# ponkrshnan/VI-HMC

Hardware: AMD Instinct MI355X
Metric: leapfrog-steps/sec/GPU (grad evals/sec) + ESS/sec, DeepONet VI-HMC (higher is better)
Workload: dtype fp32

## Files before the change

### vi-hmc_amd/csrc/vihmc_bwd_bf.hip

```cpp
#include "vihmc_internal.h"
#include "vihmc_bf16x6.h"
#include <type_traits>

namespace vihmc {

namespace {
using bf6::f32x4;
using bf6::bf16x8;
using bf6::bf16x4;
using bf6::split4;
using bf6::six;
using bf6::tr_frag;

constexpr int BB_SUB = BWD_SUB;
constexpr int BB_PITCH = bf6::PITCH;
constexpr int BB_PLANE = BB_SUB * BB_PITCH;
constexpr int BB_DP = 0;
constexpr int BB_HP = 3 * BB_PLANE;
constexpr int BB_DT = 6 * BB_PLANE;
constexpr int BB_BUF = BB_DT + BB_SUB * 16;
constexpr int BB_WPITCH = 224;
constexpr int BB_WPLANE = 100 * BB_WPITCH;
constexpr int BB_W = 2 * BB_BUF;
constexpr int BB_WT = BB_W + 3 * BB_WPLANE;
constexpr int BB_LDS = BB_WT + 100 * 16;
static_assert(BB_LDS <= 160 * 1024, "LDS");
static_assert(BB_BUF + 2 * BB_PLANE < 65536, "LDS store offsets fit the ds_write immediate");
constexpr int BB_THREADS = 1024;
constexpr int B2_HSLOTS = 2;

__device__ __forceinline__ int hslot(int r, int c4) { return c4 ^ ((r >> 2) & 3); }

__device__ __forceinline__ float act_grad_bf(int act, float h) {
#pragma clang fp contract(off)
    if (act == ACT_TANH) return 1.f - h * h;
    if (act == ACT_RELU) return h > 0.f ? 1.f : 0.f;
    return 1.f;
}
__device__ __forceinline__ float tanh_grad(float h) {
#pragma clang fp contract(off)
    return 1.f - h * h;
}
}

#if BB_STAMP
constexpr int BBS_WG = 16, BBS_SUB = 32, BBS_K = 6;
__device__ unsigned long long bb_stamps[BBS_WG][16][BBS_SUB][BBS_K];
__device__ unsigned long long bb_real[BBS_WG][2][2];
#define VIHMC_BB_STAMP(I, K)                                                                                  \
    __builtin_amdgcn_sched_barrier(0);                                                                        \
    if (samp && lane == 0 && (I) < BBS_SUB) bb_stamps[sidx][wave][(I)][(K)] = __builtin_amdgcn_s_memtime();   \
    __builtin_amdgcn_sched_barrier(0);
#else
#define VIHMC_BB_STAMP(I, K)
#endif
constexpr int BBS_NONE = 1 << 20;

__global__ __launch_bounds__(BB_THREADS, 1) void k_bwd_bf2(BwdArgs args) {
    extern __shared__ __attribute__((aligned(16))) unsigned char smw[];
    int b = blockIdx.x;
    const int per0 = args.C * args.p[0].n_wg;
    const bool second = b >= per0;
    const BwdProb P = second ? args.p[1] : args.p[0];
    if (second) b -= per0;
    const int c = b / P.n_wg;
    const int wg = b - c * P.n_wg;
    const int tid = threadIdx.x, wave = tid >> 6, lane = tid & 63, lr = lane & 15, lg = lane >> 4;
    const int NI4 = (P.n_in + 3) & ~3;
    const int hq4 = NI4 >> 2;
    const float* D = P.D + c * P.d_cs;
    const float* H = P.H + c * P.h_cs;
    const int r0 = wg * P.rows_per_wg;
    const int r1 = min(P.M, r0 + P.rows_per_wg);
    const int nsub = r1 > r0 ? (r1 - r0 + BB_SUB - 1) / BB_SUB : 0;
#if BB_STAMP
    const bool samp = second && P.has_dx && (b % 16) == 0 && b / 16 < BBS_WG;
    const int sidx = b / 16;
    if (samp && tid == 0) {
        bb_real[sidx][0][0] = __builtin_amdgcn_s_memtime();
        bb_real[sidx][0][1] = __builtin_amdgcn_s_memrealtime();
    }
#endif

    if (P.has_dx && wave < 12) {
        const float* WT = P.WT + c * P.wt_cs;
        constexpr int WTH = 768;
        constexpr int WSL = (100 * 25 + WTH - 1) / WTH;
        f32x4 wx[WSL];
#pragma unroll
        for (int v = 0; v < WSL; ++v) {
            const int idx = min(tid + WTH * v, P.n_in * 25 - 1);
            const int r = idx / 25, c4 = idx - r * 25;
            wx[v] = *reinterpret_cast<const f32x4*>(WT + (int64_t)r * P.ldw + 4 * c4);
        }
#pragma unroll
        for (int v = 0; v < WSL; ++v) {
            const int idx = tid + WTH * v;
            if (idx >= P.n_in * 25) break;
            const int r = idx / 25, c4 = idx - r * 25;
            bf16x4 p0, p1, p2;
            split4(wx[v], p0, p1, p2);
            unsigned char* o = smw + BB_W + r * BB_WPITCH + 8 * c4;
            *reinterpret_cast<bf16x4*>(o) = p0;
            *reinterpret_cast<bf16x4*>(o + BB_WPLANE) = p1;
            *reinterpret_cast<bf16x4*>(o + 2 * BB_WPLANE) = p2;
            if (c4 == 24) *reinterpret_cast<f32x4*>(smw + BB_WT + r * 16) = wx[v];
        }
    }

    if (wave >= 12) {
        const int g = __builtin_amdgcn_readfirstlane(wave - 12);
        {
            const int t = tid - 768;
            if (t < 2 * BB_SUB) {
                unsigned char* o = smw + (t >> 5) * BB_BUF + BB_HP + (t & 31) * BB_PITCH + 8 * hslot(t & 31, NI4 >> 2);
                *reinterpret_cast<unsigned short*>(o) = 0x3F80;
                *reinterpret_cast<unsigned short*>(o + BB_PLANE) = 0;
                *reinterpret_cast<unsigned short*>(o + 2 * BB_PLANE) = 0;
            }
        }
// ... 244 lines not shown
        const int tro = bf6::tr_lane_off(lr, lg);
        const int troh = (4 * lg + (lr >> 2)) * BB_PITCH + 8 * ((lr & 3) ^ lg);
        auto dw_run = [&](auto nt_c) __attribute__((always_inline)) {
            constexpr int NT = decltype(nt_c)::value;
            const int nt = NT ? NT : ntj;
            for (int i = 0; i < nsub; ++i) {
                __syncthreads();
                VIHMC_BB_STAMP(i, 0)
                const unsigned char* buf = smw + (i & 1) * BB_BUF;
                bf16x8 da[2][3], hb[2][3];
#pragma unroll
                for (int p = 0; p < 3; ++p) {
                    da[0][p] = tr_frag(buf + BB_DP + p * BB_PLANE, tro, 16 * rta);
                    da[1][p] = tr_frag(buf + BB_DP + p * BB_PLANE, tro, 16 * rtb);
                    hb[0][p] = tr_frag(buf + BB_HP + p * BB_PLANE, troh, 0);
                }
#pragma unroll
                for (int t = 0; t < 7; ++t) {
                    if (t >= nt) break;
                    if (t + 1 < nt) {
#pragma unroll
                        for (int p = 0; p < 3; ++p) hb[(t + 1) & 1][p] = tr_frag(buf + BB_HP + p * BB_PLANE, troh, 16 * (t + 1));
                    }
                    acc[0][t] = six(da[0], hb[t & 1], acc[0][t]);
                    if (t >= cb0 && t < cb1) acc[1][t] = six(da[1], hb[t & 1], acc[1][t]);
                }
#if BB_STAMP
                asm volatile("" :: "v"(acc[0][0]), "v"(acc[1][6]));
                VIHMC_BB_STAMP(i, 2)
#endif
            }
        };
        if (ntj == 7) dw_run(std::integral_constant<int, 7>{});
        else dw_run(std::integral_constant<int, 0>{});
        float* part = P.part + c * P.part_cs + (int64_t)wg * P.part_stride;
#pragma unroll
        for (int s2 = 0; s2 < 2; ++s2) {
            const int tn = s2 == 0 ? rta : rtb;
#pragma unroll
            for (int t = 0; t < 7; ++t) {
                if (t >= ntj || (s2 == 1 && (t < cb0 || t >= cb1))) continue;
                if (tn < 6 || lg == 0) *reinterpret_cast<f32x4*>(part + bwd_tile_off(tn, t, ntj, lane)) = acc[s2][t];
            }
        }
    }
#if BB_STAMP
    if (samp && tid == 0) {
        bb_real[sidx][1][0] = __builtin_amdgcn_s_memtime();
        bb_real[sidx][1][1] = __builtin_amdgcn_s_memrealtime();
    }
#endif
}

bool bwd_bf_ok(const BwdArgs& a) {
    for (int i = 0; i < a.nprob; ++i) {
        const BwdProb& p = a.p[i];
        if (p.n_out != 100 || ((p.n_in + 3) & ~3) >= 112 || (p.has_dx && p.n_in != 100)) return false;
        if ((p.ldd & 3) || (p.ldh & 3) || (p.has_dx && (p.ldw & 3)) || p.rows_per_wg % BWD_SUB) return false;
    }
    return true;
}

#if BB_STAMP
extern "C" int vihmc_debug_bb_stamps(void* stamps, size_t stamp_bytes, void* real, size_t real_bytes) {
    if (stamp_bytes != sizeof(bb_stamps) || real_bytes != sizeof(bb_real)) return -1;
    hipError_t e = hipMemcpyFromSymbol(stamps, HIP_SYMBOL(bb_stamps), stamp_bytes, 0, hipMemcpyDeviceToHost);
    if (e == hipSuccess) e = hipMemcpyFromSymbol(real, HIP_SYMBOL(bb_real), real_bytes, 0, hipMemcpyDeviceToHost);
    return (int)e;
}
#endif

hipError_t launch_bwd_bf(const BwdArgs& a, hipStream_t s) {
    if (!bwd_bf_ok(a)) return hipErrorInvalidValue;
    const int blocks = a.C * a.p[0].n_wg + (a.nprob > 1 ? a.C * a.p[1].n_wg : 0);
    hipLaunchKernelGGL(k_bwd_bf2, dim3(blocks), dim3(BB_THREADS), BB_LDS, s, a);
    return hipGetLastError();
}


}
```

### vi-hmc_amd/csrc/vihmc_internal.h

```cpp
#pragma once
#include <hip/hip_runtime.h>
#include <cstdint>
#include <vector>

#include "vihmc_diag.h"

namespace vihmc {

enum { ACT_ID = 0, ACT_TANH = 1, ACT_RELU = 2, ACT_SINE = 3 };

__device__ __forceinline__ float tanh_acc(float x) {
    const float ax = fabsf(x);
    const float u = x * x;
    float p = fmaf(u, -0.005816340912133455f, 0.020738132297992706f);
    p = fmaf(u, p, -0.053769949823617935f);
    p = fmaf(u, p, 0.13331805169582367f);
    p = fmaf(u, p, -0.33333295583724976f);
    const float small = fmaf(x * u, p, x);
    const float t = __builtin_amdgcn_exp2f(fmaf(ax, -2.885390043258667f, ax * -3.851926067000022e-08f));
    const float big = copysignf(fmaf(-2.f, t * __builtin_amdgcn_rcpf(1.f + t), 1.f), x);
    return ax < 0.625f ? small : big;
}
__device__ __forceinline__ float tanh_cr(float x) {
    const double a = fmin(fabs((double)x), 20.0);
// ... 17 lines not shown
    const double den = em + 2.0;
    const double rc = __builtin_amdgcn_rcp(den);
    const double y0 = em * rc;
    const double y = fma(fma(-y0, den, em), rc, y0);
    return copysignf((float)y, x);
}
enum { ACT_TANH_CR = 4 };
enum { MODE_FWD = 0, MODE_BWD = 1 };

constexpr int CONTRACT_OWN_PER_WG = 128;
constexpr int CONTRACT_QC = 16;
constexpr int CONTRACT_SPLIT_ROWS = 32;
constexpr int CONTRACT_SPLIT_BLOCK = 22528;
constexpr int ROWDOT_WAVES = 4;

struct RowdotProb {
    const float* A; int64_t a_cs; int32_t lda;
    const float* B; int64_t b_cs; int32_t ldb;
    float* O;       int64_t o_cs; int32_t ldo;
    const float* bias; int64_t bias_cs;
    const float* H; int64_t h_cs; int32_t ldh;
    int32_t M, Nn, K, act;
    int32_t tiles;
    int32_t ntiles;
    int32_t tpw;
};
struct RowdotArgs {
    RowdotProb p[2];
    int32_t nprob, C;
    int32_t ms0;
};



constexpr int BWD_SUB = 32;

constexpr int GATHER_SPLIT_MAX = 256;
struct BwdProb {
    const float* D;  int64_t d_cs;  int32_t ldd;
    const float* WT; int64_t wt_cs; int32_t ldw;
    const float* H;  int64_t h_cs;  int32_t ldh;
    float* Dout;     int64_t o_cs;
    float* part;     int64_t part_cs; int32_t part_stride;
    int32_t M, n_out, n_in, act, has_dx;
    int32_t rows_per_wg, n_wg;
};
struct BwdArgs {
    BwdProb p[2];
    int32_t nprob, C;
};
hipError_t launch_bwd(const BwdArgs& a, int nti, hipStream_t s);
bool bwd_bf_ok(const BwdArgs& a);
hipError_t launch_bwd_bf(const BwdArgs& a, hipStream_t s);

constexpr int BWD_CHAIN_MAXL = 12;
struct BwdChainLayer {
    const float* H; int64_t h_cs; int32_t ldh;
    int32_t n_in, n_out;
    int32_t act;
    int64_t part_off; int32_t part_stride;
};
struct BwdChainNet {
    BwdChainLayer L[BWD_CHAIN_MAXL];
    int32_t nl, M, n_wg;
    int32_t tanh_all;
    const float* D; int64_t d_cs; int32_t ldd;
    float* dwpart; int64_t dwpart_cs;
    const unsigned char* wtimg; int64_t wtimg_cs;
};
struct BwdChainArgs {
    BwdChainNet net[2];
    int32_t C;
};
bool bwd_chain_ok(const BwdChainArgs& a);
hipError_t launch_bwd_chain(const BwdChainArgs& a, hipStream_t s);
int bwd_chain_rows();

constexpr int GUARD_MAXC = 256;
struct ChainBits {
    uint32_t w[GUARD_MAXC / 32];
};
__host__ __device__ inline bool chain_bit(const ChainBits& b, int c) {
    return c < GUARD_MAXC && ((b.w[c >> 5] >> (c & 31)) & 1u) != 0u;
}

struct ContractProb {
    const float* Own; int64_t own_cs; int32_t ldown;
    const float* Q;   int64_t q_cs;   int32_t ldq;
    const float* Y;   int32_t ldy; int64_t y_cs;
    float* gout;      int64_t gout_cs; int32_t ldg;
    const float* b0;  int64_t b0_cs;
    float* out;       int64_t out_cs; int32_t ldout; int64_t out_chunk_stride;
    double* stats;    int64_t stats_cs;
    int32_t Mo, Mq, W;
    int32_t o_tiles, q_chunks, q_per_chunk;
    int32_t with_stats, write_s;
    int32_t load_g;
    int32_t masked;
    int32_t xcd_group;
    int32_t bf16x6;
    const unsigned char* qimg; int64_t qimg_cs;
    float gscale;
    int32_t sel; ChainBits bits;
};

constexpr int MOMENTS_TILE_N = 64;
// ... 256 lines not shown
```

### vi-hmc_amd/csrc/vihmc_plan.hip

```cpp
#include <algorithm>
#include <cmath>
#include <cstring>
#include <string>
#include <vector>

#include "vihmc.h"
#include "vihmc_internal.h"
#include <cstdlib>
#include <cstdio>

using namespace vihmc;

namespace {

thread_local std::string g_err;
constexpr size_t CANARY_BYTES = 4096;

int fail(const std::string& msg, int code = 1) {
    g_err = msg;
    return code;
}

#define HIPCHK(expr)                                                                              \
    do {                                                                                          \
// ... 103 lines not shown
    float* gT = nullptr;
    int64_t gT_cs = 0;
    int ldgT = 0;
    unsigned char* qsplitA = nullptr;
    int64_t qsplitA_cs = 0;
    unsigned char* qsplitB = nullptr;
    int64_t qsplitB_cs = 0;
    bool img_by_fwd = false;
    float* partB = nullptr;
    int64_t partB_cs = 0;
    int qchunksB = 1, qperB = 32;
    int qchunksA = 1, qperA = 32;
    float* partA = nullptr;
    int64_t partA_cs = 0;
    ReduceJob* jobsA = nullptr;
    int lenA = 0;
    double* stats = nullptr;
    int64_t stats_cs = 0;
    int nwavesA = 0;
    ReduceJob* jobsB = nullptr;
    ReduceJob* jobsW = nullptr;
    ReduceJob* jobsWt = nullptr;
    uint8_t* gsamp = nullptr;
    int n_jobsW = 0, max_lenW = 0, lenB = 0;
    int spanA = 0, spanB = 0, spanW = 0, spanWt = 0;

    std::vector<int32_t> fmap_host;

    MlpArgs mlp{};
    int maxw = 0;

    int timing_on = 0;
    int timing_every = 1;
    int64_t n_evals = 0;
    std::vector<hipEvent_t> ev_pool;
    std::vector<int> ev_cls;
    std::vector<int> ev_nl;
    size_t ev_used = 0;

    std::vector<std::pair<int, hipGraphExec_t>> graphs;
    hipStream_t cap_stream = nullptr;
    unsigned char* wimg = nullptr;
    int64_t wimg_cs = 0;
    unsigned char* wtimg = nullptr;
    int64_t wtimg_cs = 0;
    int32_t* smap_timg = nullptr;
    int32_t* smap_timgf = nullptr;
    int fwd_wimg = 1;
    int fwd_in0 = 1;
    int skip_zt = 1;
    int fuse_scatter = 1;
    int mlp_fast = 1;
    int bwd_chain = 1;
    int gram = 1, gram_min_chains = 4;
    bool gram_alloc = false;
    __bf16* gya = nullptr;
    __bf16* gyb = nullptr;
    int64_t gya_plane = 0, gyb_plane = 0;
    int gya_ld = 0, gyb_ld = 0, gNG = 0, gS = 0, gSL = 0, gPT = 0, gSB = 1, gSLB = 1, gSt = 1, gSLt = 1;
    int gStc = 1, gSLtc = 1;
    float* gtt_part = nullptr;
    int64_t gtt_cs = 0;
    float* gtb_part = nullptr;
    int64_t gtb_cs = 0;
    double* ggt_part = nullptr;
    int64_t ggt_part_cs = 0;
    int gSb = 1, gSLb = 1;
    double* ggb_part = nullptr;
    int64_t ggb_part_cs = 0;
    float* gtb_sum = nullptr;
    int64_t gtbs_cs = 0;
    float* ggt = nullptr;
    double* ggt64 = nullptr;
    unsigned char* ggb = nullptr;
    unsigned char* ggb3 = nullptr;
    double* gstats = nullptr;
    int64_t gstats_cs = 0;
    int gram_center = 1;
    int gram_pair2 = 0;
    bool centre_stale = true;
    int tanh_cr = 1;
    int debug_dz = 0;
    float* dzb_snap = nullptr;
    float* dzt_snap = nullptr;
    double* msse_part = nullptr;
    double* msse_stats = nullptr;
    unsigned char* cimgB = nullptr;
    unsigned char* cimgT = nullptr;
    float* cB0 = nullptr;
    double* ccol = nullptr;
    double* cysq = nullptr;
    float* cpk = nullptr;
    unsigned char* cwimg = nullptr;
    unsigned char* cwtimg = nullptr;
    float* save_pk = nullptr;
    unsigned char* save_wimg = nullptr;
    unsigned char* save_wtimg = nullptr;
    float* ght_part = nullptr;
    float* ghb_part = nullptr;
    int64_t ght_cs = 0, ghb_cs = 0;
    float* ght = nullptr;
    unsigned char* ghb = nullptr;
    unsigned char* ghb3 = nullptr;
    bool last_gram = false;
    int last_gram_chains = 0;
    int64_t n_grad_calls = 0;
    int64_t n_gram_calls = 0;
    int64_t n_gram_chain_evals = 0;
    int gram_guard = 1;
    int y_masked = 0;
    int64_t lik_count = 0;
    float* fit_dev = nullptr;
    double* ysq_dev = nullptr;
    double* gcol = nullptr;
    double* ysq_part = nullptr;
    float* fit_host = nullptr;
    hipEvent_t fit_ev[2] = {nullptr, nullptr};
    int snap_C[2] = {0, 0};
    int64_t n_snap = 0;
    bool capturing = false;
    bool timg_live = false;
    bool last_bwd_chain = false;
    float *g_theta = nullptr, *g_logp = nullptr, *g_grad = nullptr;
    int graph_on = -1;
    int fwd_bf16x6 = [] {
        const char* e = std::getenv("VIHMC_FWD_BF16");
        return e ? (std::atoi(e) != 0 ? 1 : 0) : 1;
    }();
    int bwd_bf16x6 = [] {
        const char* e = std::getenv("VIHMC_BWD_BF16");
        return e ? (std::atoi(e) != 0 ? 1 : 0) : 1;
    }();
    int contract_bf16x6 = [] {
        const char* e = std::getenv("VIHMC_CONTRACT_BF16");
        return e ? (std::atoi(e) != 0 ? 1 : 0) : 1;
    }();

    template <typename T>
    int alloc(T** p, int64_t n) {
        void* v = nullptr;
        const size_t sz = std::max<int64_t>(n, 1) * sizeof(T);
        hipError_t e = guard_pages ? vmm_alloc(&v, sz + (canary ? CANARY_BYTES : 0))
                                   : hipMalloc(&v, sz + (canary ? CANARY_BYTES : 0));
        if (e != hipSuccess) return fail(std::string("hipMalloc(") + std::to_string(sz) + "): " + hipGetErrorString(e), (int)e);
        e = hipMemset(v, 0, sz);
        if (e != hipSuccess) return fail(std::string("hipMemset: ") + hipGetErrorString(e), (int)e);
        if (canary) {
            e = hipMemset(static_cast<unsigned char*>(v) + sz, 0xA5, CANARY_BYTES);
            if (e != hipSuccess) return fail(std::string("hipMemset: ") + hipGetErrorString(e), (int)e);
            canaries.push_back(static_cast<unsigned char*>(v) + sz);
        }
        if (!guard_pages) allocs.push_back(v);
        bytes += sz;
        *p = static_cast<T*>(v);
        return 0;
    }
    template <typename T>
    int upload(T** p, const T* host, int64_t n) {
        if (int rc = alloc(p, n)) return rc;
        HIPCHK(hipMemcpy(*p, host, n * sizeof(T), hipMemcpyHostToDevice));
        return 0;
    }
    ~vihmc_plan() {
        for (hipEvent_t e : fit_ev)
            if (e) (void)hipEventDestroy(e);
        if (fit_host) (void)hipHostFree(fit_host);
        for (auto& g : graphs) (void)hipGraphExecDestroy(g.second);
        if (cap_stream) (void)hipStreamDestroy(cap_stream);
        for (void* p : allocs) (void)hipFree(p);
        if (!vmm.empty()) (void)hipDeviceSynchronize();
        for (auto& b : vmm) {
            (void)hipMemUnmap(b.base, b.mapped);
            (void)hipMemRelease(b.h);
        }
        for (hipEvent_t e : ev_pool) (void)hipEventDestroy(e);
// ... 556 lines not shown
                if (cost < best) best = cost, qa = q;
            }
        }
        p->qperA = (int)(((int64_t)cdiv(p->N, qa) + CONTRACT_SPLIT_ROWS - 1) / CONTRACT_SPLIT_ROWS * CONTRACT_SPLIT_ROWS);
        p->qchunksA = cdiv(p->N, p->qperA);
        if (p->qchunksA > 1) {
            p->partA_cs = r64((int64_t)p->qchunksA * p->P * p->ldz);
            if (int rc = p->alloc(&p->partA, p->partA_cs * C)) return rc;
        }
        int qc = std::max(1, (int)std::lround((double)og_a * p->qchunksA / og_b));
        if (p->W == 100) {
            qc = std::max(1, (int)std::lround(256.0 / ((double)C * cdiv(p->N, CONTRACT_BF_B_OWN))));
            qc = std::min(qc, std::max(1, cdiv(p->P, CONTRACT_B_MIN_Q)));
            qc = std::min(qc, cdiv(p->P, CONTRACT_SPLIT_ROWS));
        }
        p->qperB = (int)(((int64_t)cdiv(p->P, qc) + CONTRACT_SPLIT_ROWS - 1) / CONTRACT_SPLIT_ROWS * CONTRACT_SPLIT_ROWS);
        p->qchunksB = cdiv(p->P, p->qperB);
        p->partB_cs = r64((int64_t)p->qchunksB * p->N * p->ldz);
        if (int rc = p->alloc(&p->partB, p->partB_cs * C)) return rc;
        p->nwavesA = p->qchunksA * og_a * 8;
        p->stats_cs = 2 * (int64_t)p->nwavesA;
        if (int rc = p->alloc(&p->stats, p->stats_cs * C)) return rc;
        if (int rc = p->alloc(&p->lik_buf, C)) return rc;
        if (int rc = p->alloc(&p->lp_part, (int64_t)C * GATHER_SPLIT_MAX)) return rc;
        if (int rc = p->alloc(&p->fin_cnt, C)) return rc;
    }
    {
        ReduceJob jb{};
        jb.src = p->partB;
        jb.in_cs = p->partB_cs;
        jb.part_stride = (int64_t)p->N * p->ldz;
        jb.n_parts = p->qchunksB;
        jb.len = p->N * p->ldz;
        jb.dst = p->nets[0].delta[0];
        jb.dst_cs = p->nets[0].delta_cs;
        p->lenB = jb.len;
        p->spanB = reduce_span(&jb, 1);
        if (int rc = p->upload(&p->jobsB, &jb, 1)) return rc;
        if (p->qchunksA > 1) {
            ReduceJob ja{};
            ja.src = p->partA;
            ja.in_cs = p->partA_cs;
            ja.part_stride = (int64_t)p->P * p->ldz;
            ja.n_parts = p->qchunksA;
            ja.len = p->P * p->ldz;
            ja.dst = p->nets[1].delta[0];
            ja.dst_cs = p->nets[1].delta_cs;
            p->lenA = ja.len;
            const ReduceJob both[2] = {jb, ja};
            p->spanA = reduce_span(both, 2);
            if (int rc = p->upload(&p->jobsA, both, 2)) return rc;
        }
        std::vector<ReduceJob> jw, jt;
        std::vector<char> tiled[2];
        for (int net = 0; net < 2; ++net) tiled[net].assign(p->nets[net].L.size(), 0);
        const int maxl = (int)std::max(p->nets[0].L.size(), p->nets[1].L.size());
        for (int i = 0; i < maxl; ++i) {
            BwdArgs ba{};
            int js[2] = {-1, -1};
            for (int net = 0; net < 2; ++net) {
                const Net& n = p->nets[net];
                const int j = (int)n.L.size() - 1 - i;
                if (j < 0) continue;
                js[net] = j;
                const LayerPk& L = n.L[j];
                BwdProb& q = ba.p[ba.nprob++];
                q.ldd = q.ldw = L.ldo;
                q.ldh = L.ldi;
                q.n_out = L.n_out;
                q.n_in = L.n_in;
                q.has_dx = j >= 1;
                q.rows_per_wg = L.rows_per_chunk;
            }
            if (bwd_bf_ok(ba))
                for (int net = 0; net < 2; ++net)
                    if (js[net] >= 0) tiled[net][js[net]] = 1;
        }
        for (int net = 0; net < 2; ++net) {
            Net& n = p->nets[net];
            for (size_t li = 0; li < n.L.size(); ++li) {
                const LayerPk& L = n.L[li];
                ReduceJob j{};
                j.src = n.dwpart + L.part_off;
                j.in_cs = n.dwpart_cs;
                j.part_stride = L.part_stride;
                j.n_parts = L.n_chunks;
                j.len = L.n_out * L.ldi + L.n_out;
                j.dst = p->gp + L.wp;
                j.dst_cs = p->dp;
                j.samp = p->gsamp && L.n_chunks >= REDUCE_GROUP_MIN ? p->gsamp + L.wp : nullptr;
                p->max_lenW = std::max(p->max_lenW, j.len);
                jw.push_back(j);
                if (tiled[net][li]) {
                    j.tiled = 1;
                    j.ntj = (L.ldi + 16) >> 4;
                    j.len = bwd_tile_floats(j.ntj);
                    j.n_out = L.n_out;
                    j.n_in = L.n_in;
                    j.ldi = L.ldi;
                    p->max_lenW = std::max(p->max_lenW, j.len);
                }
                jt.push_back(j);
            }
        }
        p->n_jobsW = (int)jw.size();
        p->spanW = reduce_span(jw.data(), (int)jw.size());
        p->spanWt = reduce_span(jt.data(), (int)jt.size());
// ... 375 lines not shown
        q.Y = p->gT;
        q.ldy = p->contract_bf16x6 && p->W == 100 ? gt_block_rows(p) : p->ldgT;
        q.y_cs = p->gT_cs;
        q.load_g = 1;
        q.bf16x6 = p->W == 100 ? p->contract_bf16x6 : 0;
        q.qimg = p->qsplitB;
        q.qimg_cs = p->qsplitB_cs;
        q.xcd_group = ((int64_t)C * p->qchunksB) % 8 == 0 ? 1 : 0;
        q.b0 = p->packed;
        q.b0_cs = p->dp;
        q.sel = mixed ? 1 : 0;
        q.bits = resid;
        q.out = p->partB;
        q.out_cs = p->partB_cs;
        q.ldout = p->ldz;
        q.out_chunk_stride = (int64_t)p->N * p->ldz;
        q.stats = p->stats;
        q.Mo = p->N;
        q.Mq = p->P;
        q.W = p->W;
        q.o_tiles = cdiv(p->N, q.bf16x6 ? CONTRACT_BF_B_OWN : CONTRACT_OWN_PER_WG);
        q.q_chunks = p->qchunksB;
        q.q_per_chunk = p->qperB;
        q.with_stats = 0;
        const float v = std::max(p->lik.tau_out, 1e-6f);
        q.gscale = p->lik.loss == VIHMC_LOSS_NLL ? -1.f / v : -p->lik.tau_out;
        if (q.bf16x6 && !p->img_by_fwd)
            HIPCHK(launch_split_blocks(q.Q, q.q_cs, q.ldq, p->P, p->qsplitB, p->qsplitB_cs, C, s));
        hipEvent_t stop = nullptr;
        if (int rc = p->timing_begin(VIHMC_T_CONTRACT_B, s, &stop)) return rc;
        HIPCHK(launch_contract(q, C, true, s));
        if (stop) HIPCHK(hipEventRecord(stop, s));
        const ChainBits* only = mixed ? &resid : nullptr;
        if (p->qchunksA > 1) HIPCHK(launch_reduce(p->jobsA, 2, p->spanA, C, s, nullptr, only));
        else HIPCHK(launch_reduce(p->jobsB, 1, p->spanB, C, s, nullptr, only));
        }

        if (p->debug_dz) {
            if (!p->dzb_snap) {
                if (int rc = p->alloc(&p->dzb_snap, b.delta_cs * p->maxC)) return rc;
                if (int rc = p->alloc(&p->dzt_snap, t.delta_cs * p->maxC)) return rc;
            }
            HIPCHK(hipMemcpyAsync(p->dzb_snap, b.delta[0], sizeof(float) * b.delta_cs * C, hipMemcpyDeviceToDevice, s));
            HIPCHK(hipMemcpyAsync(p->dzt_snap, t.delta[0], sizeof(float) * t.delta_cs * C, hipMemcpyDeviceToDevice, s));
        }
        int cur[2] = {0, 0};
        const int maxl = (int)std::max(b.L.size(), t.L.size());
        hipEvent_t bwd_stop = nullptr;
        if (int rc = p->timing_begin(VIHMC_T_BWD, s, &bwd_stop, maxl)) return rc;
        BwdChainArgs ca{};
        const bool chain = p->bwd_chain && p->bwd_bf16x6 && p->timg_live && bwd_chain_args(p, C, ca);
        if (chain) HIPCHK(launch_bwd_chain(ca, s));
        p->last_bwd_chain = chain;
        for (int i = 0; i < (chain ? 0 : maxl); ++i) {
            BwdArgs ba{};
            ba.C = C;
            int nti = 1;
            for (int net = 0; net < 2; ++net) {
                Net& n = p->nets[net];
                const int j = (int)n.L.size() - 1 - i;
                if (j < 0) continue;
                const LayerPk& L = n.L[j];
                BwdProb& q = ba.p[ba.nprob++];
                q.D = n.delta[cur[net]];
                q.d_cs = n.delta_cs;
                q.ldd = L.ldo;
                q.WT = p->packed + L.wt;
                q.wt_cs = p->dp;
                q.ldw = L.ldo;
                q.H = j == 0 ? n.input : n.act + n.h_off[j - 1];
                q.h_cs = j == 0 ? 0 : n.act_cs;
                q.ldh = L.ldi;
                q.Dout = n.delta[cur[net] ^ 1];
                q.o_cs = n.delta_cs;
                q.part = n.dwpart + L.part_off;
                q.part_cs = n.dwpart_cs;
                q.part_stride = (int32_t)L.part_stride;
                q.M = n.rows;
                q.n_out = L.n_out;
                q.n_in = L.n_in;
                q.act = j >= 1 ? n.L[j - 1].act : 0;
                q.has_dx = j >= 1;
                q.rows_per_wg = L.rows_per_chunk;
                q.n_wg = L.n_chunks;
                nti = std::max(nti, nt_of(L.n_in));
            }
            if (ba.nprob == 1) ba.p[1] = ba.p[0];
            if (p->bwd_bf16x6 && bwd_bf_ok(ba)) HIPCHK(launch_bwd_bf(ba, s));
            else HIPCHK(launch_bwd(ba, nti, s));
            for (int net = 0; net < 2; ++net) {
                const int j = (int)p->nets[net].L.size() - 1 - i;
                if (j >= 1) cur[net] ^= 1;
            }
        }
        if (bwd_stop) HIPCHK(hipEventRecord(bwd_stop, s));
        HIPCHK(launch_reduce(p->bwd_bf16x6 ? p->jobsWt : p->jobsW, p->n_jobsW, p->bwd_bf16x6 ? p->spanWt : p->spanW,
                             C, s, &stats_job));
    }
    HIPCHK(launch_gather_prior(p->gp, p->dp, p->smap_w, theta, p->K, p->prior_mu, p->prior_iv, p->prior_const,
                               p->lik.prior_scale, p->lik_buf, C, logp, want_grad ? grad : nullptr, p->lp_part, p->fin_cnt, s,
                               want_grad ? leap : nullptr));
    if (snap)
        if (int rc = guard_snapshot(p, C, s)) return rc;
    return 0;
}

int deeponet_predict_moments(vihmc_plan* p, const float* theta, int C, float* logp, double* sum1, double* sum2,
                             int accumulate, double* sse_rows, hipStream_t s) {
    if (C < 1 || C > p->maxC) return fail("C must be in [1, max_chains]");
    const int p_tiles = cdiv(p->P, MOMENTS_TILE_P);
    const int n_tiles = cdiv(p->N, MOMENTS_TILE_N);
    if (!p->msse_part) {
        if (int rc = p->alloc(&p->msse_part, (int64_t)p->maxC * p_tiles * p->N)) return rc;
        if (int rc = p->alloc(&p->msse_stats, (int64_t)p->maxC * n_tiles * 2)) return rc;
    }
    ++p->n_evals;
    hipEvent_t stop = nullptr;
    if (int rc = p->timing_begin(VIHMC_T_EVAL, s, &stop)) return rc;
    const ScatterImg si = scatter_img(p);
    HIPCHK(launch_scatter(p->packed, p->dp, C, theta, p->K, p->smap_w, p->smap_wt, s, p->img_by_scatter ? &si : nullptr));
    p->img_by_fwd = false;
    p->timg_live = p->img_by_scatter && p->wtimg;
    if (int rc = deeponet_forward_layers(p, C, s, false, false)) return rc;
    Net& b = p->nets[0];
    Net& t = p->nets[1];
    MomentsProb m{};
    m.Zb = b.act + b.h_off.back();
    m.zb_cs = b.act_cs;
    m.Zt = t.act + t.h_off.back();
    m.zt_cs = t.act_cs;
    m.ldz = p->ldz;
    m.Y = p->y;
    m.ldy = p->P;
    m.masked = p->y_masked;
    m.b0 = p->packed;
    m.b0_cs = p->dp;
    m.sum1 = sum1;
    m.sum2 = sum2;
    m.accumulate = accumulate ? 1 : 0;
    m.part = p->msse_part;
    m.sse_rows = sse_rows;
    m.stats = p->msse_stats;
// ... 553 lines not shown
    });
}

int vihmc_plan_kind(const vihmc_plan* p) { return p ? p->kind : -1; }
int64_t vihmc_plan_n_params(const vihmc_plan* p) { return p ? p->D : -1; }
int vihmc_plan_K(const vihmc_plan* p) { return p ? p->K : -1; }
int vihmc_plan_max_chains(const vihmc_plan* p) { return p ? p->maxC : -1; }
int64_t vihmc_plan_device_bytes(const vihmc_plan* p) { return p ? p->bytes : -1; }

int vihmc_timing_enable(vihmc_plan* p, int which, int on) {
    if (!p) return fail("null plan");
    if (which < -1 || which >= VIHMC_T_COUNT) return fail("timing class out of range");
    const int bits = which < 0 ? (1 << VIHMC_T_COUNT) - 1 : 1 << which;
    p->timing_on = on ? (p->timing_on | bits) : (p->timing_on & ~bits);
    p->ev_used = 0;
    p->ev_cls.clear();
    p->ev_nl.clear();
    return 0;
}

int vihmc_timing_read_class(vihmc_plan* p, int which, double* total_ms, int64_t* launches) {
    if (!p || !total_ms || !launches) return fail("null argument");
    double t = 0.0;
    int64_t n = 0;
    for (size_t i = 0; i + 1 < p->ev_used; i += 2) {
        if (which >= 0 && p->ev_cls[i / 2] != which) continue;
        HIPCHK(hipEventSynchronize(p->ev_pool[i + 1]));
        float ms = 0.f;
        HIPCHK(hipEventElapsedTime(&ms, p->ev_pool[i], p->ev_pool[i + 1]));
        t += ms;
        n += p->ev_nl[i / 2];
    }
    *total_ms = t;
    *launches = n;
    return 0;
}

int vihmc_timing_read(vihmc_plan* p, double* total_ms, int64_t* launches) {
    const int rc = vihmc_timing_read_class(p, -1, total_ms, launches);
    if (p && rc == 0) {
        p->ev_used = 0;
        p->ev_cls.clear();
    }
    return rc;
}

int vihmc_timing_reset(vihmc_plan* p) {
    if (!p) return fail("null plan");
    p->ev_used = 0;
    p->ev_cls.clear();
    return 0;
}

#define OPTION_KEYS "fwd_bf16x6, contract_bf16x6, bwd_bf16x6, graph, timing_every, fwd_wimg, fwd_in0, skip_zt, fuse_scatter, img_scatter, mlp_fast, bwd_chain, gram, gram_active, gram_center, gram_pair2, tanh_cr, debug_dz, gram_min_chains, gram_guard, grad_evals, gram_evals, gram_chains, gram_chain_evals, y_masked, lik_count"

int vihmc_plan_option(vihmc_plan* p, const char* key, int value) {
    if (!p || !key) return fail("null argument");
    const std::string k(key);
    if (k == "fwd_bf16x6") p->fwd_bf16x6 = value ? 1 : 0;
    else if (k == "contract_bf16x6") p->contract_bf16x6 = value ? 1 : 0;
    else if (k == "bwd_bf16x6") p->bwd_bf16x6 = value ? 1 : 0;
    else if (k == "graph") p->graph_on = value ? 1 : 0;
    else if (k == "fwd_wimg") p->fwd_wimg = value ? 1 : 0;
    else if (k == "fwd_in0") p->fwd_in0 = value ? 1 : 0;
    else if (k == "skip_zt") p->skip_zt = value ? 1 : 0;
    else if (k == "timing_every") {
        p->timing_every = std::max(1, value);
        return 0;
    }
    else if (k == "fuse_scatter") p->fuse_scatter = value ? 1 : 0;
    else if (k == "img_scatter") p->img_by_scatter = value && p->smap_img;
    else if (k == "mlp_fast") p->mlp_fast = value ? 1 : 0;
    else if (k == "bwd_chain") p->bwd_chain = value ? 1 : 0;
    else if (k == "gram") p->gram = value ? 1 : 0;
    else if (k == "gram_min_chains") p->gram_min_chains = std::max(1, value);
    else if (k == "gram_guard") {
        p->gram_guard = std::max(0, value);
        p->n_snap = 0;
    }
    else if (k == "y_masked" || k == "lik_count") {
        if (p->kind != 0) return fail("plan option '" + k + "': DeepONet plans only");
        if (k == "y_masked") p->y_masked = value ? 1 : 0;
        else if (value < 0 || (double)value > (double)p->N * (double)p->P) return fail("lik_count must be in [0, N P]");
        else p->lik_count = value;
    }
    else if (k == "gram_active") return fail("plan option 'gram_active' is read-only");
    else if (k == "debug_dz") {
        p->debug_dz = value ? 1 : 0;
        return 0;
    }
    else if (k == "tanh_cr") {
        p->tanh_cr = value ? 1 : 0;
        p->centre_stale = true;
    }
    else if (k == "gram_pair2") {
        if (value < 0 || value > 2) return fail("gram_pair2: 0, 1 or 2");
        p->gram_pair2 = value;
    }
    else if (k == "gram_center") {
        if ((value ? 1 : 0) != p->gram_center) {
            p->gram_center = value ? 1 : 0;
            if (int rc = gram_images(p, nullptr)) return rc;
            HIPCHK(hipDeviceSynchronize());
        }
    }
    else if (k == "grad_evals" || k == "gram_evals") {
        p->n_grad_calls = p->n_gram_calls = p->n_gram_chain_evals = 0;
        return 0;
    }
    else return fail("unknown plan option '" + k + "' (" OPTION_KEYS ")");
    for (auto& g : p->graphs) (void)hipGraphExecDestroy(g.second);
    p->graphs.clear();
    return 0;
}

int vihmc_plan_get_option(const vihmc_plan* p, const char* key, int* value) {
    if (!p || !key || !value) return fail("null argument");
    const std::string k(key);
    if (k == "fwd_bf16x6") *value = p->fwd_bf16x6;
    else if (k == "contract_bf16x6") *value = p->contract_bf16x6 && p->W == 100;
    else if (k == "bwd_bf16x6") *value = p->bwd_bf16x6;
    else if (k == "graph") *value = p->graph_on;
    else if (k == "fwd_wimg") *value = p->fwd_wimg;
    else if (k == "fwd_in0") *value = p->kind == 0 && fused_forward_ok(p) && fused_input_ok(p);
    else if (k == "skip_zt") *value = p->skip_zt;
    else if (k == "timing_every") *value = p->timing_every;
    else if (k == "fuse_scatter") *value = p->fuse_scatter;
    else if (k == "img_scatter") *value = p->img_by_scatter ? 1 : 0;
    else if (k == "mlp_fast") *value = p->mlp_fast && p->kind == 1 && mlp_bnn_fast_ok(p->mlp);
    else if (k == "bwd_chain") *value = p->bwd_chain | (p->last_bwd_chain ? 2 : 0);
    else if (k == "gram") *value = (p->gram && p->gram_alloc ? 1 : 0) | (p->last_gram ? 2 : 0);
    else if (k == "gram_min_chains") *value = p->gram_min_chains;
    else if (k == "gram_active") *value = gram_on(p) ? 1 : 0;
    else if (k == "gram_center") *value = p->gram_center;
    else if (k == "gram_pair2") *value = p->gram_pair2;
    else if (k == "tanh_cr") *value = p->tanh_cr;
    else if (k == "debug_dz") *value = p->debug_dz;
    else if (k == "grad_evals") *value = (int)std::min<int64_t>(p->n_grad_calls, INT32_MAX);
    else if (k == "gram_evals") *value = (int)std::min<int64_t>(p->n_gram_calls, INT32_MAX);
    else if (k == "gram_chains") *value = p->last_gram_chains;
    else if (k == "gram_chain_evals") *value = (int)std::min<int64_t>(p->n_gram_chain_evals, INT32_MAX);
    else if (k == "gram_guard") *value = p->gram_guard;
    else if (k == "y_masked") *value = p->y_masked;
    else if (k == "lik_count") *value = (int)std::min<double>(lik_count(p), INT32_MAX);
    else return fail("unknown plan option '" + k + "' (" OPTION_KEYS ")");
    return 0;
}

int vihmc_plan_check_canaries(vihmc_plan* p, int64_t* corrupted) {
    return guarded([&]() -> int {
        if (!p || !corrupted) return fail("null argument");
        if (!p->canary) return fail("vihmc_plan_check_canaries: plan created without VIHMC_CANARY=1");
        HIPCHK(hipDeviceSynchronize());
        std::vector<unsigned char> h(CANARY_BYTES);
        int64_t bad = 0;
        for (unsigned char* c : p->canaries) {
            HIPCHK(hipMemcpy(h.data(), c, CANARY_BYTES, hipMemcpyDeviceToHost));
            for (unsigned char v : h) bad += v != 0xA5;
        }
        *corrupted = bad;
        return 0;
    });
}

int vihmc_plan_debug_copy(vihmc_plan* p, const char* name, void* dst, int64_t* bytes) {
    return guarded([&]() -> int {
        if (!p || !name || !bytes) return fail("null argument");
        if (p->kind != 0) return fail("vihmc_plan_debug_copy: DeepONet plans only");
        const std::string k(name);
        const void* src = nullptr;
        int64_t n = 0;
        const Net& b = p->nets[0];
        const Net& t = p->nets[1];
        const int64_t C = p->maxC;
        if (k == "dzb") src = b.delta[0], n = 4 * b.delta_cs * C;
        else if (k == "dzt") src = t.delta[0], n = 4 * t.delta_cs * C;
        else if (k == "act_b") src = b.act, n = 4 * b.act_cs * C;
        else if (k == "act_t") src = t.act, n = 4 * t.act_cs * C;
        else if (k == "bimg") src = p->qsplitA, n = p->qsplitA_cs * C;
        else if (k == "timg") src = p->qsplitB, n = p->qsplitB_cs * C;
        else if (k == "gram_tb") src = p->gtb_part, n = 4 * p->gtb_cs * C;
        else if (k == "gram_gt_part") src = p->ggt_part, n = 8 * p->ggt_part_cs * C;
        else if (k == "gram_gb_part") src = p->ggb_part, n = 8 * p->ggb_part_cs * C;
// ... 51 lines not shown
```

Measured before the change: 11800.

## Fuse per-layer bf16x6 backward launches into one persistent multi-layer kernel

Result: faster. 12030, median of 6 (+2.0%).

```diff
diff --git a/profiles/kstats_per_step.py b/profiles/kstats_per_step.py
--- /dev/null
+++ b/profiles/kstats_per_step.py
@@ -0,0 +1,32 @@
+import csv
+import re
+import sys
+
+
+def load(path):
+    d = {}
+    with open(path) as f:
+        for r in csv.DictReader(f):
+            name = re.sub(r"\(.*", "", r["Name"]).replace("vihmc::", "").replace("void ", "")
+            d[name] = (int(r["Calls"]), float(r["TotalDurationNs"]) / 1e3)
+    return d
+
+
+def main():
+    a, b, steps = load(sys.argv[1]), load(sys.argv[2]), int(sys.argv[3])
+    top = int(sys.argv[4]) if len(sys.argv) > 4 else 14
+    rows = []
+    for n, (c1, t1) in b.items():
+        c0, t0 = a.get(n, (0, 0.0))
+        if c1 > c0:
+            rows.append((n, (c1 - c0) / steps, (t1 - t0) / steps, (t1 - t0) / (c1 - c0)))
+    rows.sort(key=lambda r: -r[2])
+    tot = sum(r[2] for r in rows)
+    print(f"kernel time per HMC step {tot:.1f} us in {sum(r[1] for r in rows):.1f} launches")
+    print(f"{'kernel':44s} {'per step':>9s} {'us/step':>10s} {'avg_us':>9s} {'pct':>6s}")
+    for n, c, t, avg in rows[:top]:
+        print(f"{n[:44]:44s} {c:9.2f} {t:10.1f} {avg:9.2f} {100 * t / tot:6.2f}")
+
+
+if __name__ == "__main__":
+    main()
diff --git a/vi-hmc_amd/csrc/vihmc_bwd_bf.hip b/vi-hmc_amd/csrc/vihmc_bwd_bf.hip
--- a/vi-hmc_amd/csrc/vihmc_bwd_bf.hip
+++ b/vi-hmc_amd/csrc/vihmc_bwd_bf.hip
@@ -56,16 +56,10 @@
 #endif
 constexpr int BBS_NONE = 1 << 20;
 
-__global__ __launch_bounds__(BB_THREADS, 1) void k_bwd_bf2(BwdArgs args) {
+__device__ __forceinline__ void bwd_bf2_layer(const BwdProb& P, const int c, const int wg, const int b, const bool second,
+                                              const int tid) {
     extern __shared__ __attribute__((aligned(16))) unsigned char smw[];
-    int b = blockIdx.x;
-    const int per0 = args.C * args.p[0].n_wg;
-    const bool second = b >= per0;
-    const BwdProb P = second ? args.p[1] : args.p[0];
-    if (second) b -= per0;
-    const int c = b / P.n_wg;
-    const int wg = b - c * P.n_wg;
-    const int tid = threadIdx.x, wave = tid >> 6, lane = tid & 63, lr = lane & 15, lg = lane >> 4;
+    const int wave = tid >> 6, lane = tid & 63, lr = lane & 15, lg = lane >> 4;
     const int NI4 = (P.n_in + 3) & ~3;
     const int hq4 = NI4 >> 2;
     const float* D = P.D + c * P.d_cs;
@@ -416,6 +410,37 @@
 #endif
 }
 
+__global__ __launch_bounds__(BB_THREADS, 1) void k_bwd_bf2(BwdArgs args) {
+    int b = blockIdx.x;
+    const int per0 = args.C * args.p[0].n_wg;
+    const bool second = b >= per0;
+    const BwdProb P = second ? args.p[1] : args.p[0];
+    if (second) b -= per0;
+    const int c = b / P.n_wg;
+    bwd_bf2_layer(P, c, b - c * P.n_wg, b, second, threadIdx.x);
+}
+
+__global__ __launch_bounds__(BB_THREADS, 1) void k_bwd_bf2_layers(BwdLayersArgs args) {
+    int b = blockIdx.x;
+    const int per0 = args.C * args.p[0][0].n_wg;
+    const int net = b >= per0 ? 1 : 0;
+    if (net) b -= per0;
+    const int n_wg = args.p[net][0].n_wg;
+    const int c = b / n_wg;
+    const int wg = b - c * n_wg;
+    const int nk = args.nk[net];
+    for (int k = 0; k < nk; ++k) {
+        if (k) {
+            if (threadIdx.x < 512) asm volatile("s_waitcnt vmcnt(0)" ::: "memory");
+            __syncthreads();
+        }
+        int tid = threadIdx.x;
+        asm volatile("" : "+v"(tid));
+        __builtin_assume(tid >= 0 && tid < BB_THREADS);
+        bwd_bf2_layer(args.p[net][k], c, wg, b, net != 0, tid);
+    }
+}
+
 bool bwd_bf_ok(const BwdArgs& a) {
     for (int i = 0; i < a.nprob; ++i) {
         const BwdProb& p = a.p[i];
@@ -434,6 +459,29 @@
 }
 #endif
 
+bool bwd_layers_ok(const BwdLayersArgs& a) {
+    for (int net = 0; net < 2; ++net) {
+        if (a.nk[net] < 1 || a.nk[net] > BWD_LAYERS_MAXK) return false;
+        for (int k = 0; k < a.nk[net]; ++k) {
+            const BwdProb& q = a.p[net][k];
+            BwdArgs one{};
+            one.p[0] = q;
+            one.nprob = 1;
+            if (!q.has_dx || !bwd_bf_ok(one)) return false;
+            if (q.rows_per_wg != a.p[net][0].rows_per_wg || q.n_wg != a.p[net][0].n_wg || q.M != a.p[net][0].M) return false;
+            if (k && (q.D != a.p[net][k - 1].Dout || q.d_cs != a.p[net][k - 1].o_cs)) return false;
+        }
+    }
+    return true;
+}
+
+hipError_t launch_bwd_bf_layers(const BwdLayersArgs& a, hipStream_t s) {
+    if (!bwd_layers_ok(a)) return hipErrorInvalidValue;
+    const int blocks = a.C * (a.p[0][0].n_wg + a.p[1][0].n_wg);
+    hipLaunchKernelGGL(k_bwd_bf2_layers, dim3(blocks), dim3(BB_THREADS), BB_LDS, s, a);
+    return hipGetLastError();
+}
+
 hipError_t launch_bwd_bf(const BwdArgs& a, hipStream_t s) {
     if (!bwd_bf_ok(a)) return hipErrorInvalidValue;
     const int blocks = a.C * a.p[0].n_wg + (a.nprob > 1 ? a.C * a.p[1].n_wg : 0);
diff --git a/vi-hmc_amd/csrc/vihmc_internal.h b/vi-hmc_amd/csrc/vihmc_internal.h
--- a/vi-hmc_amd/csrc/vihmc_internal.h
+++ b/vi-hmc_amd/csrc/vihmc_internal.h
@@ -93,6 +93,15 @@
 hipError_t launch_bwd(const BwdArgs& a, int nti, hipStream_t s);
 bool bwd_bf_ok(const BwdArgs& a);
 hipError_t launch_bwd_bf(const BwdArgs& a, hipStream_t s);
+
+constexpr int BWD_LAYERS_MAXK = 11;
+struct BwdLayersArgs {
+    BwdProb p[2][BWD_LAYERS_MAXK];
+    int32_t nk[2], C;
+};
+static_assert(sizeof(BwdLayersArgs) <= 4096, "kernel-argument segment");
+bool bwd_layers_ok(const BwdLayersArgs& a);
+hipError_t launch_bwd_bf_layers(const BwdLayersArgs& a, hipStream_t s);
 
 constexpr int BWD_CHAIN_MAXL = 12;
 struct BwdChainLayer {
diff --git a/vi-hmc_amd/csrc/vihmc_plan.hip b/vi-hmc_amd/csrc/vihmc_plan.hip
--- a/vi-hmc_amd/csrc/vihmc_plan.hip
+++ b/vi-hmc_amd/csrc/vihmc_plan.hip
@@ -179,6 +179,7 @@
     int fuse_scatter = 1;
     int mlp_fast = 1;
     int bwd_chain = 1;
+    int bwd_layers = 1;
     int gram = 1, gram_min_chains = 4;
     bool gram_alloc = false;
     __bf16* gya = nullptr;
@@ -248,6 +249,8 @@
     bool capturing = false;
     bool timg_live = false;
     bool last_bwd_chain = false;
+    bool last_bwd_layers = false;
+    std::vector<char> bwd_tiled[2];
     float *g_theta = nullptr, *g_logp = nullptr, *g_grad = nullptr;
     int graph_on = -1;
     int fwd_bf16x6 = [] {
@@ -910,7 +913,7 @@
             if (int rc = p->upload(&p->jobsA, both, 2)) return rc;
         }
         std::vector<ReduceJob> jw, jt;
-        std::vector<char> tiled[2];
+        std::vector<char>(&tiled)[2] = p->bwd_tiled;
         for (int net = 0; net < 2; ++net) tiled[net].assign(p->nets[net].L.size(), 0);
         const int maxl = (int)std::max(p->nets[0].L.size(), p->nets[1].L.size());
         for (int i = 0; i < maxl; ++i) {
@@ -1392,42 +1395,64 @@
         const bool chain = p->bwd_chain && p->bwd_bf16x6 && p->timg_live && bwd_chain_args(p, C, ca);
         if (chain) HIPCHK(launch_bwd_chain(ca, s));
         p->last_bwd_chain = chain;
+        auto layer_prob = [&](int net, int j, int cur) {
+            Net& n = p->nets[net];
+            const LayerPk& L = n.L[j];
+            BwdProb q{};
+            q.D = n.delta[cur];
+            q.d_cs = n.delta_cs;
+            q.ldd = L.ldo;
+            q.WT = p->packed + L.wt;
+            q.wt_cs = p->dp;
+            q.ldw = L.ldo;
+            q.H = j == 0 ? n.input : n.act + n.h_off[j - 1];
+            q.h_cs = j == 0 ? 0 : n.act_cs;
+            q.ldh = L.ldi;
+            q.Dout = n.delta[cur ^ 1];
+            q.o_cs = n.delta_cs;
+            q.part = n.dwpart + L.part_off;
+            q.part_cs = n.dwpart_cs;
+            q.part_stride = (int32_t)L.part_stride;
+            q.M = n.rows;
+            q.n_out = L.n_out;
+            q.n_in = L.n_in;
+            q.act = j >= 1 ? n.L[j - 1].act : 0;
+            q.has_dx = j >= 1;
+            q.rows_per_wg = L.rows_per_chunk;
+            q.n_wg = L.n_chunks;
+            return q;
+        };
+        bool layers = !chain && p->bwd_layers && p->bwd_bf16x6;
+        BwdLayersArgs la{};
+        la.C = C;
+        for (int net = 0; net < 2 && layers; ++net) {
+            const int nl = (int)p->nets[net].L.size();
+            layers = nl >= 2 && nl - 1 <= BWD_LAYERS_MAXK;
+            for (int j = nl - 1; j >= 1 && layers; --j) {
+                layers = p->bwd_tiled[net][j] != 0;
+                la.p[net][la.nk[net]] = layer_prob(net, j, la.nk[net] & 1);
+                ++la.nk[net];
+            }
+        }
+        layers = layers && bwd_layers_ok(la);
+        if (layers) HIPCHK(launch_bwd_bf_layers(la, s));
+        p->last_bwd_layers = layers;
         for (int i = 0; i < (chain ? 0 : maxl); ++i) {
             BwdArgs ba{};
             ba.C = C;
             int nti = 1;
+            bool bf = true;
             for (int net = 0; net < 2; ++net) {
                 Net& n = p->nets[net];
                 const int j = (int)n.L.size() - 1 - i;
-                if (j < 0) continue;
-                const LayerPk& L = n.L[j];
-                BwdProb& q = ba.p[ba.nprob++];
-                q.D = n.delta[cur[net]];
-                q.d_cs = n.delta_cs;
-                q.ldd = L.ldo;
-                q.WT = p->packed + L.wt;
-                q.wt_cs = p->dp;
-                q.ldw = L.ldo;
-                q.H = j == 0 ? n.input : n.act + n.h_off[j - 1];
-                q.h_cs = j == 0 ? 0 : n.act_cs;
-                q.ldh = L.ldi;
-                q.Dout = n.delta[cur[net] ^ 1];
-                q.o_cs = n.delta_cs;
-                q.part = n.dwpart + L.part_off;
-                q.part_cs = n.dwpart_cs;
-                q.part_stride = (int32_t)L.part_stride;
-                q.M = n.rows;
-                q.n_out = L.n_out;
-                q.n_in = L.n_in;
-                q.act = j >= 1 ? n.L[j - 1].act : 0;
-                q.has_dx = j >= 1;
-                q.rows_per_wg = L.rows_per_chunk;
-                q.n_wg = L.n_chunks;
-                nti = std::max(nti, nt_of(L.n_in));
+                if (j < 0 || (layers && j >= 1)) continue;
+                ba.p[ba.nprob++] = layer_prob(net, j, layers ? la.nk[net] & 1 : cur[net]);
+                bf = bf && p->bwd_tiled[net][j];
+                nti = std::max(nti, nt_of(n.L[j].n_in));
             }
             if (ba.nprob == 1) ba.p[1] = ba.p[0];
-            if (p->bwd_bf16x6 && bwd_bf_ok(ba)) HIPCHK(launch_bwd_bf(ba, s));
-            else HIPCHK(launch_bwd(ba, nti, s));
+            if (ba.nprob && p->bwd_bf16x6 && bf) HIPCHK(launch_bwd_bf(ba, s));
+            else if (ba.nprob) HIPCHK(launch_bwd(ba, nti, s));
             for (int net = 0; net < 2; ++net) {
                 const int j = (int)p->nets[net].L.size() - 1 - i;
                 if (j >= 1) cur[net] ^= 1;
@@ -2087,7 +2112,7 @@
     return 0;
 }
 
-#define OPTION_KEYS "fwd_bf16x6, contract_bf16x6, bwd_bf16x6, graph, timing_every, fwd_wimg, fwd_in0, skip_zt, fuse_scatter, img_scatter, mlp_fast, bwd_chain, gram, gram_active, gram_center, gram_pair2, tanh_cr, debug_dz, gram_min_chains, gram_guard, grad_evals, gram_evals, gram_chains, gram_chain_evals, y_masked, lik_count"
+#define OPTION_KEYS "fwd_bf16x6, contract_bf16x6, bwd_bf16x6, graph, timing_every, fwd_wimg, fwd_in0, skip_zt, fuse_scatter, img_scatter, mlp_fast, bwd_chain, bwd_layers, gram, gram_active, gram_center, gram_pair2, tanh_cr, debug_dz, gram_min_chains, gram_guard, grad_evals, gram_evals, gram_chains, gram_chain_evals, y_masked, lik_count"
 
 int vihmc_plan_option(vihmc_plan* p, const char* key, int value) {
     if (!p || !key) return fail("null argument");
@@ -2107,6 +2132,7 @@
     else if (k == "img_scatter") p->img_by_scatter = value && p->smap_img;
     else if (k == "mlp_fast") p->mlp_fast = value ? 1 : 0;
     else if (k == "bwd_chain") p->bwd_chain = value ? 1 : 0;
+    else if (k == "bwd_layers") p->bwd_layers = value ? 1 : 0;
     else if (k == "gram") p->gram = value ? 1 : 0;
     else if (k == "gram_min_chains") p->gram_min_chains = std::max(1, value);
     else if (k == "gram_guard") {
@@ -2164,6 +2190,7 @@
     else if (k == "img_scatter") *value = p->img_by_scatter ? 1 : 0;
     else if (k == "mlp_fast") *value = p->mlp_fast && p->kind == 1 && mlp_bnn_fast_ok(p->mlp);
     else if (k == "bwd_chain") *value = p->bwd_chain | (p->last_bwd_chain ? 2 : 0);
+    else if (k == "bwd_layers") *value = p->bwd_layers | (p->last_bwd_layers ? 2 : 0);
     else if (k == "gram") *value = (p->gram && p->gram_alloc ? 1 : 0) | (p->last_gram ? 2 : 0);
     else if (k == "gram_min_chains") *value = p->gram_min_chains;
     else if (k == "gram_active") *value = gram_on(p) ? 1 : 0;
```
